# StefanDenn3r/Unsupervised_Anomaly_Detection_Brain_MRI

Hardware: AMD Instinct MI355X
Metric: MRI slices/sec VAE train step (128x128, bs=64) (higher is better)
Workload: dtype bf16x3; 1 GPU; BASELINE.json configs[1]: VAE 128x128x1 slices, batch 64 per GPU, fwd + bwd + TF-Adam (lr 1e-4, beta1 0.5), dropout 0.2, inter_res 8, zDim 128; global_batch=64, per_gpu_batch=64, parallelism=single

## Files before the change

unsupervised_anomaly_detection_brain_mri_amd/csrc/uad_conv16s.inc:

```

__device__ __forceinline__ float sum32_half(float v) {
    v += __uint_as_float(dpp_u32<0xB1>(__float_as_uint(v)));
    v += __uint_as_float(dpp_u32<0x4E>(__float_as_uint(v)));
    v += __uint_as_float(dpp_u32<0x141>(__float_as_uint(v)));
    v += __uint_as_float(dpp_u32<0x140>(__float_as_uint(v)));
    v += __uint_as_float((unsigned)__builtin_amdgcn_update_dpp(0, (int)__float_as_uint(v), 0x142, 0xa, 0xf, false));
    return v;
}
__device__ __forceinline__ bool sum32_valid(int lane) { return (lane & 16) != 0; }

__device__ __forceinline__ float xhalf_sum(float v) {
    const auto r = __builtin_amdgcn_permlane32_swap(__float_as_uint(v), __float_as_uint(v), false, false);
    return __uint_as_float(r[0]) + __uint_as_float(r[1]);
}
__device__ __forceinline__ unsigned xhalf_or(unsigned v) {
    const auto r = __builtin_amdgcn_permlane32_swap(v, v, false, false);
    return r[0] | r[1];
}

#ifndef UAD_D16S_NACC
#define UAD_D16S_NACC 1
#endif
template <int TH, int TW, int CST, int WGM, int WGN, int NPL = 2>
constexpr size_t conv5_d16s_lds_bytes(int epi) {
// ... 428 lines not shown
                    const int c = 8 * (r >> 2) + 4 * lh + (r & 3);
                    const float wfc = s_par[2 * BN + c];
                    fr[c] = t0;
                    fr[32 + c] = wfc * t1;
                    fr[64 + c] = wfc * t2;
                }
            }
        }
        float r0 = rec, r1 = dbf;
        r0 = sum32_half(r0); r1 = sum32_half(r1);
        if (lane == 16) { fr[96] = r1; fr[97] = r0; }
        __syncthreads();
        static_assert(TW == 16 && (TH == 8 || TH == 16), "partial-sum slots of the fused final epilogue are 8 x 16 tiles");
        const int slots_x = d.WS / 16;
        const size_t tile = ((size_t)n * (d.HS / 8) + ty0 / 8) * slots_x + tx0 / 16;
        if (tid < FL) {
            float t = 0.f;
#pragma unroll
            for (int w = 0; w < NW; ++w) t += s_red[w * FL + tid];
            if (tid == 97) a.ep.fin_rec_partial[tile] = t;
            else if (want_grad) a.ep.fin_red_partial[tile * 97 + tid] = t;
            if constexpr (TH == 16) {
                if (tid == 97) a.ep.fin_rec_partial[tile + slots_x] = 0.f;
                else if (want_grad) a.ep.fin_red_partial[(tile + slots_x) * 97 + tid] = 0.f;
            }
        }
        return;
    }
    if constexpr (BWD) {
        float* fr = s_red + wave * FL;
#pragma unroll
        for (int r = 0; r < 16; ++r) {
            const float t1 = sum32_half(s1[r]), t2 = sum32_half(s2[r]);
            if (l31 == 16) {
                const int c = 8 * (r >> 2) + 4 * lh + (r & 3);
                fr[c] = t1;
                fr[32 + c] = t2;
            }
        }
        __syncthreads();
// ... 63 lines not shown
```

unsupervised_anomaly_detection_brain_mri_amd/csrc/uad_gemm.hip:

```cpp
#include <type_traits>
#include "uad_kernels.h"
#include <hip/hip_ext.h>
#include <stdio.h>
#include <stdlib.h>
#include <string.h>
#include <map>
#include <array>
#include <string>
#include <vector>

#include "uad_gemm_common.h"

namespace {

constexpr int XF_LDS_CH = 512;

template <int BM, int BN, int BK, int WGM, int WGN, int KIND>
__global__ void __launch_bounds__(64 * WGM * WGN) conv_gemm_kernel(const ConvGemmArgs a) {
    constexpr int NT = 64 * WGM * WGN;
    constexpr int WTM = BM / WGM, WTN = BN / WGN;
    constexpr int FM = WTM / 32, FN = WTN / 32;
    static_assert(WTM % 32 == 0 && WTN % 32 == 0, "wave tile must be a multiple of the 32x32 MFMA");
    static_assert(BK % 8 == 0, "BK multiple of 8");
    constexpr int NKK = BK / 8;
// ... 2614 lines not shown
    for (int i = 0; i < n; ++i) v8 = v8 && pd.count[i] % 8 == 0 && pd.cb[i] % 8 == 0 && pd.cs[i] % 8 == 0;
    if (v8) hipLaunchKernelGGL(pack_weights_bf16_v8_kernel<3>, dim3((unsigned)((total / 8 + 255) / 256), 2), dim3(256), 0, st, params, w3_f, w3_d, pd);
    else hipLaunchKernelGGL(pack_weights_bf16_3p_kernel, dim3((unsigned)((total + 255) / 256)), dim3(256), 0, st, params, w3_f, w3_d, pd);
}

namespace {
void run_plan(const GemmPlan& p, ConvGemmArgs& a, bool f_type, float* ws, hipStream_t st) {
    const UadConvDesc& d = a.d;
    a.nsplit = 1; a.out_elems = p.out_elems;
    a.dbg = 0; a.dbgbuf = nullptr;
    if (p.path == PATH_SPATIAL) {
        float* out = a.Out;
        if (p.nsplit > 1) { a.Out = ws; a.nsplit = p.nsplit; a.out_final = out; }
        if (!(p.nsplit > 1 && p.inkernel && a.Wp16)) a.sk_counter = nullptr;
        dim3 grid((d.HS / p.sc.TH) * (d.WS / p.sc.TW), d.N, (a.Nn / p.sc.BN) * p.nsplit);
        if (a.Wp16) {
            if (f_type) {
                if (a.npl == 3) {
                    if (p.sc.BN == 64) {
                        if (a.xf.fb_bits || a.xf.fb_dxhat) { fprintf(stderr, "uad: final-backward on load runs on the 32-column instance (CA <= 32)\n"); abort(); }
                        if (a.xf.scale) launch_conv5_f16_v<8, 8, 16, 2, 2, 0, true, 3>(a, grid, st); else launch_conv5_f16_v<8, 8, 16, 2, 2, 0, false, 3>(a, grid, st);
                    } else launch_conv5_f16<8, 16, 16, 4, 1, 3>(a, grid, st);
                } else
                if (p.sc.BN == 64) launch_conv5_f16<8, 8, 32, 2, 2>(a, grid, st);
                else launch_conv5_f16<8, 16, 16, 4, 1>(a, grid, st);
            } else {
                const int cst = (a.CA % p.nsplit == 0) ? a.CA / p.nsplit : 0;
                constexpr bool seq = true;
                const bool lp = seq && conv5_d16s_takes(a);
                if (lp && ((p.sc.BN == 64 && (cst == 128 || cst == 64 || cst == 32)) || (p.sc.BN == 32 && (cst == 64 || cst == 32)))) launch_conv5_d16s_any(a, grid, p.sc.BN, cst, st);
                else if (a.npl == 3) { fprintf(stderr, "uad: a bf16x6 launch reached a kernel without the three-plane form (x6_route decides before run_plan)\n"); abort(); }
                else
                if (p.sc.BN == 64) {
                    if (seq && cst == 128) launch_conv5_d16<8, 8, 128, 2, 2>(a, grid, st);
                    else if (seq && cst == 64) launch_conv5_d16<8, 8, 64, 2, 2>(a, grid, st);
                    else if (seq && cst == 32) launch_conv5_d16<8, 8, 32, 2, 2>(a, grid, st);
                    else launch_conv5_bf16<8, 8, 32, 2, 2, KIND_D>(a, grid, st);
                } else if (seq && cst == 64) launch_conv5_d16<8, 16, 64, 4, 1>(a, grid, st);
                else if (seq && cst == 32) launch_conv5_d16<8, 16, 32, 4, 1>(a, grid, st);
                else if (p.sc.CK == 32) launch_conv5_bf16<8, 16, 32, 4, 1, KIND_D>(a, grid, st);
                else launch_conv5_bf16<8, 16, 16, 4, 1, KIND_D>(a, grid, st);
            }
        } else if (f_type) {
            if (p.sc.BN == 64) UAD_SPATIAL_LAUNCH((conv5_f_kernel<8, 8, 32, 2, 2>), grid, dim3(256), 0, st, a);
            else UAD_SPATIAL_LAUNCH((conv5_f_kernel<8, 16, 16, 4, 1>), grid, dim3(256), 0, st, a);
        } else {
            if (p.sc.BN == 64 && a.ep.kind != UAD_EPI_FINAL) UAD_SPATIAL_LAUNCH((conv5_d_kernel<8, 8, 32, 2, 2>), grid, dim3(256), 0, st, a);
            else if (p.sc.CK == 32 && a.ep.kind == UAD_EPI_FINAL && p.nsplit == 1 && a.Nn == 32) UAD_SPATIAL_LAUNCH((conv5_d_kernel<8, 16, 32, 4, 1, true>), grid, dim3(256), 0, st, a);
            else if (a.ep.kind == UAD_EPI_FINAL) { fprintf(stderr, "uad: fused final epilogue asked of an exact-fp32 launch that cannot run it (check uad_conv_d_can_fuse_final_f32 first)\n"); abort(); }
            else if (p.sc.CK == 32) UAD_SPATIAL_LAUNCH((conv5_d_kernel<8, 16, 32, 4, 1>), grid, dim3(256), 0, st, a);
            else UAD_SPATIAL_LAUNCH((conv5_d_kernel<8, 16, 16, 4, 1>), grid, dim3(256), 0, st, a);
        }
        if (p.nsplit > 1 && !a.sk_counter) {
            dim3 g2((p.out_rows + 63) / 64, (a.Nn + 63) / 64);
            hipLaunchKernelGGL(splitk_epilogue_kernel, g2, dim3(256), 0, st, ws, p.nsplit, p.out_elems, p.out_rows, a.Nn, a.ep, out);
        }
        return;
    }
    const int classes = f_type ? 1 : d.S * d.S;
    if (p.path == PATH_SPLITK) {
        float* out = a.Out;
        a.Out = ws; a.nsplit = p.nsplit;
        if (f_type) launch_gemm<KIND_F>(a, classes, st); else launch_gemm<KIND_D>(a, classes, st);
        dim3 grid((p.out_rows + 63) / 64, (a.Nn + 63) / 64);
        hipLaunchKernelGGL(splitk_epilogue_kernel, grid, dim3(256), 0, st, ws, p.nsplit, p.out_elems, p.out_rows, a.Nn, a.ep, out);
        return;
    }
// ... 244 lines not shown
```

unsupervised_anomaly_detection_brain_mri_amd/csrc/uad_kernels.h:

```cpp
#pragma once
#include <hip/hip_runtime.h>
#include <stdint.h>

struct UadConvDesc {
    int N;
    int HB, WB, CB;
    int HS, WS, CS;
    int KS, S, P;
};

struct UadXform {
    const float* scale = nullptr;
    const float* shift = nullptr;
    float alpha = 1.f;
    float mult = 1.f;
    const float* fb_dxhat = nullptr;
    const float* fb_wf = nullptr;
    const unsigned* fb_bits = nullptr;
};

enum { UAD_EPI_BIAS = 0, UAD_EPI_BWD_ACT = 1, UAD_EPI_FINAL = 2 };

struct UadGemmWs { float* ptr; size_t floats; unsigned* counters; int ncounters; };

// ... 7 lines not shown
    const float* eshift;
    float ealpha;
    float emult;
    float* colpart;
    const float* fin_wf;
    const float* fin_bf;
    const float* fin_x;
    float* fin_xhat;
    float* fin_l1;
    float* fin_rec_partial;
    float* fin_red_partial;
    float* fin_dc;
    unsigned* fin_bits;
    float* fin_dxhat;
    float fin_inv_batch;
};

void uad_launch_conv_f(const UadConvDesc& d, const float* big_in, UadXform xf, const float* W,
                       float* small_out, UadEpilogue ep, hipStream_t st, const float* Wpacked = nullptr,
                       UadGemmWs ws = UadGemmWs{nullptr, 0}, const unsigned short* Wp16 = nullptr, long long w16_plane = 0,
                       bool generic_bf16x3 = false, int planes16 = 2);
void uad_launch_conv_d(const UadConvDesc& d, const float* small_in, UadXform xf, const float* W,
                       float* big_out, UadEpilogue ep, hipStream_t st, const float* Wpacked = nullptr,
                       UadGemmWs ws = UadGemmWs{nullptr, 0}, const unsigned short* Wp16 = nullptr, long long w16_plane = 0,
                       bool generic_bf16x3 = false, int planes16 = 2);
void uad_launch_pack_weights_bf16(const float* params, unsigned short* w16_f, unsigned short* w16_d, const long long* offs,
                                  const int* cbs, const int* css, const int* taps, int n, hipStream_t st);
void uad_launch_pack_weights_bf16_3p(const float* params, unsigned short* w3_f, unsigned short* w3_d, const long long* offs,
                                     const int* cbs, const int* css, const int* taps, int n, hipStream_t st);
bool uad_conv_k3_takes(const UadConvDesc& d, bool f_type);
// ... 12 lines not shown
void uad_conv_plan_query(const UadConvDesc& d, bool f_type, bool have_pack, size_t ws_floats, int ncounters, int planes16, bool inst_ok, long long* out);
void uad_conv_w_plan_query(const UadConvDesc& d, bool math_bf16x3, int planes16, bool fbb, bool xa, bool xs, bool generic_bf16x3, bool defer_reduce, long long* out);
size_t uad_conv_w_partial_floats(const UadConvDesc& d);
bool uad_conv_w_supports_fb_bits(const UadConvDesc& d, bool math_bf16x3);
void uad_launch_conv_w(const UadConvDesc& d, const float* big, UadXform xfb, const float* small, UadXform xfs,
                       float* dW, float* partial, hipStream_t st, bool math_bf16x3 = false,
                       hipStream_t reduce_st = nullptr, hipEvent_t ev = nullptr, bool generic_bf16x3 = false, bool defer_reduce = false, int planes16 = 2);
void uad_launch_conv_w_reduce(const UadConvDesc& d, float* dW, float* partial, hipStream_t st, bool math_bf16x3);

void uad_launch_reduce_partials(const float* partial, int S, int L, float scale, float* out, hipStream_t st);
void uad_launch_bn_grad_finalize(const float* colpart, int T, int C, const float* gamma, float rstd,
                                 float* dgamma, float* dbeta, float* dbias, hipStream_t st, float* scratch = nullptr);
size_t uad_bn_grad_finalize_scratch_floats(int C);
void uad_launch_final_gradfin(const float* red, int C, const float* gamma, float rstd, float* dwf, float* dbf, float* dgamma, float* dbeta,
                              float* dbias, hipStream_t st);
void uad_launch_colsum(const float* g, int rows, int C, float* out, float* scratch, hipStream_t st);
size_t uad_colsum_scratch_floats(int rows, int C);

void uad_launch_conv_first_fwd(const UadConvDesc& d, const float* x, const float* W, const float* bias,
                               float* out, hipStream_t st);
size_t uad_conv_first_wgrad_partial_floats(const UadConvDesc& d);
void uad_launch_conv_first_wgrad(const UadConvDesc& d, const float* x, const float* g, float* dW,
                                 float* partial, hipStream_t st);

struct UadFinalArgs {
    int N, H, W, C;
    const float* c_last;
    const float* scale;
    const float* shift;
    float alpha;
// ... 123 lines not shown
void uad_launch_spatial_z_fwd(const float* c, const float* gamma, const float* beta, float rs0, float alpha, const float* mask, int rows,
                              int C, float* z, hipStream_t st);
int uad_spatial_z_bwd_blocks(int rows);
void uad_launch_spatial_z_bwd(const float* dz, const float* c, const float* gamma, const float* beta, float rs0, float alpha,
                              const float* mask, int rows, int C, float* dc, float* colpart, hipStream_t st);
struct UadRngJob { float* out; int per_sample; int kind; float rate; int stream; };
void uad_launch_rng_fill(const UadRngJob* jobs, int njobs, int n, unsigned long long seed, unsigned long long step, long long sample0,
                         hipStream_t st);
void uad_launch_clock_probe(unsigned long long* out, unsigned long long ticks, hipStream_t st);
void uad_launch_gather_slices(const float* src, const int* idx, int n, long long slice_elems, float* out, hipStream_t st);
void uad_launch_gather_mask(const unsigned char* labels, const int* idx, int n, long long slice_px, const unsigned char* lut,
                            float* out, hipStream_t st);
void uad_launch_mul(const float* x, const float* mask, float* y, size_t n, hipStream_t st);
void uad_launch_loss_finalize(const float* rec_partial, int n, int n_vae, int bps, const float* kl_per_sample,
                              float inv_batch, float rec_scale, float* rec_per_sample, float* scalars, hipStream_t st);

void uad_launch_optim(int kind, float* p, const float* g, float* s1, float* s2, size_t n, float lr, float momentum, float decay, float eps,
                      float gscale, hipStream_t st, const unsigned* fault = nullptr);
void uad_launch_adam(float* p, const float* g, float* m, float* v, size_t n, float lr_t, float beta1, float beta2,
                     float eps, float gscale, hipStream_t st, const unsigned* fault = nullptr);

void uad_launch_residual(const float* x, const float* xr, const float* mask, int n, int hw, int pos_only,
                         float prior_thresh, float* out, float* l1err, hipStream_t st);
```

unsupervised_anomaly_detection_brain_mri_amd/csrc/uad_misc.hip:

```cpp
#include "uad_kernels.h"
#include <stdint.h>

namespace {

__device__ __forceinline__ float wave_sum(float v) {
#pragma unroll
    for (int o = 32; o > 0; o >>= 1) v += __shfl_xor(v, o);
    return v;
}

typedef float v4f_nt __attribute__((ext_vector_type(4)));
template <int JL, int SL>
__global__ void __launch_bounds__(JL * SL) reduce_partials4_kernel(const float* __restrict__ partial, int S, int L, float scale, float* __restrict__ out) {
    __shared__ v4f_nt red[SL][JL];
    const int jl = threadIdx.x % JL, sl = threadIdx.x / JL;
    const int j4 = blockIdx.x * JL + jl, L4 = L >> 2;
    v4f_nt a0 = {0.f, 0.f, 0.f, 0.f}, a1 = a0, a2 = a0, a3 = a0;
    if (j4 < L4) {
        const v4f_nt* p = reinterpret_cast<const v4f_nt*>(partial) + j4;
        int s = sl;
        for (; s + 3 * SL < S; s += 4 * SL) {
            const v4f_nt v0 = __builtin_nontemporal_load(p + (size_t)s * L4), v1 = __builtin_nontemporal_load(p + (size_t)(s + SL) * L4);
            const v4f_nt v2 = __builtin_nontemporal_load(p + (size_t)(s + 2 * SL) * L4), v3 = __builtin_nontemporal_load(p + (size_t)(s + 3 * SL) * L4);
            a0 += v0; a1 += v1; a2 += v2; a3 += v3;
        }
        for (; s < S; s += SL) a0 += __builtin_nontemporal_load(p + (size_t)s * L4);
    }
    red[sl][jl] = (a0 + a1) + (a2 + a3);
    __syncthreads();
    if (sl == 0 && j4 < L4) {
        v4f_nt t = red[0][jl];
#pragma unroll
        for (int k = 1; k < SL; ++k) t += red[k][jl];
        reinterpret_cast<v4f_nt*>(out)[j4] = t * scale;
    }
}

template <int SL>
__global__ void __launch_bounds__(64 * SL) reduce_partials_kernel(const float* __restrict__ partial, int S, int L,
                                                                  float scale, float* __restrict__ out, int nt) {
    __shared__ float red[SL][64];
    const int jl = threadIdx.x & 63, sl = threadIdx.x >> 6;
    const int j = blockIdx.x * 64 + jl;
    float a0 = 0.f, a1 = 0.f, a2 = 0.f, a3 = 0.f;
    if (j < L) {
        int s = sl;
        if (nt) {
            for (; s + 3 * SL < S; s += 4 * SL) {
                a0 += __builtin_nontemporal_load(partial + (size_t)s * L + j);
                a1 += __builtin_nontemporal_load(partial + (size_t)(s + SL) * L + j);
                a2 += __builtin_nontemporal_load(partial + (size_t)(s + 2 * SL) * L + j);
                a3 += __builtin_nontemporal_load(partial + (size_t)(s + 3 * SL) * L + j);
            }
        }
        for (; s + 3 * SL < S; s += 4 * SL) {
            a0 += partial[(size_t)s * L + j];
            a1 += partial[(size_t)(s + SL) * L + j];
            a2 += partial[(size_t)(s + 2 * SL) * L + j];
            a3 += partial[(size_t)(s + 3 * SL) * L + j];
        }
        for (; s < S; s += SL) a0 += partial[(size_t)s * L + j];
    }
    red[sl][jl] = (a0 + a1) + (a2 + a3);
    __syncthreads();
    if (sl == 0 && j < L) {
        float t = 0.f;
#pragma unroll
        for (int k = 0; k < SL; ++k) t += red[k][jl];
        out[j] = t * scale;
    }
}

__global__ void __launch_bounds__(1024) bn_grad_finalize_kernel(const float* __restrict__ colpart, int T, int C,
                                                                const float* __restrict__ gamma, float rstd,
                                                                float* __restrict__ dgamma, float* __restrict__ dbeta,
                                                                float* __restrict__ dbias) {
    __shared__ float red[2][32][33];
    const int cl = threadIdx.x & 31, g = threadIdx.x >> 5;
// ... 61 lines not shown
        if (dbias) dbias[c] = gamma[c] * rstd * a1;
    }
}

__global__ void __launch_bounds__(256) final_gradfin_kernel(const float* __restrict__ red, int C, const float* __restrict__ gamma, float rstd,
                                                            float* __restrict__ dwf, float* __restrict__ dbf, float* __restrict__ dgamma,
                                                            float* __restrict__ dbeta, float* __restrict__ dbias) {
    for (int c = threadIdx.x; c < C; c += 256) {
        const float s1 = red[C + c], s2 = red[2 * C + c];
        dwf[c] = red[c];
        if (dbeta) dbeta[c] = s1;
        if (dgamma) dgamma[c] = s2 * rstd;
        if (dbias) dbias[c] = gamma[c] * rstd * s1;
    }
    if (threadIdx.x == 0) dbf[0] = red[3 * C];
}

__global__ void __launch_bounds__(256) colsum_kernel(const float* __restrict__ g, int rows, int C, int rows_per_chunk,
                                                     float* __restrict__ out) {
    __shared__ float red[8][33];
    const int cl = threadIdx.x & 31, rl = threadIdx.x >> 5;
    const int c = blockIdx.x * 32 + cl;
    const int r0 = blockIdx.y * rows_per_chunk;
    const int r1 = min(r0 + rows_per_chunk, rows);
    float s = 0.f;
    if (c < C)
        for (int r = r0 + rl; r < r1; r += 8) s += g[(size_t)r * C + c];
    red[rl][cl] = s;
    __syncthreads();
    if (rl == 0 && c < C) {
// ... 482 lines not shown
    __syncthreads();
    const int cq = threadIdx.x & 7, slot = threadIdx.x >> 3;
    first_dgrad_class<0, 0>(sg, W, cq, slot, sout);
    first_dgrad_class<0, 1>(sg, W, cq, slot, sout);
    first_dgrad_class<1, 0>(sg, W, cq, slot, sout);
    first_dgrad_class<1, 1>(sg, W, cq, slot, sout);
    __syncthreads();
    const int y = threadIdx.x >> 4, x = threadIdx.x & 15;
    first_dgrad_store(e, ((size_t)n * d.HB + ty0 + y) * d.WB + tx0 + x, sout[threadIdx.x]);
}

__global__ void __launch_bounds__(256) loss_finalize_kernel(const float* __restrict__ rec_partial, int n, int n_vae,
                                                            int bps, const float* __restrict__ kl, float inv_batch,
                                                            float rec_scale, float* __restrict__ rec_per_sample,
                                                            float* __restrict__ scalars) {
    __shared__ float sr[256], sc[256], sk[256];
    float ar = 0.f, ac = 0.f, ak = 0.f;
    for (int i = threadIdx.x; i < n; i += 256) {
        float r = 0.f;
        for (int b = 0; b < bps; ++b) r += rec_partial[(size_t)i * bps + b];
        rec_per_sample[i] = r;
        if (i < n_vae) { ar += r; if (kl) ak += kl[i]; }
        else ac += r;
    }
    sr[threadIdx.x] = ar;
    sc[threadIdx.x] = ac;
    sk[threadIdx.x] = ak;
    __syncthreads();
    if (threadIdx.x == 0) {
        float tr = 0.f, tc = 0.f, tk = 0.f;
        for (int i = 0; i < 256; ++i) { tr += sr[i]; tc += sc[i]; tk += sk[i]; }
        scalars[0] = rec_scale * (tr + tc) * inv_batch;
        scalars[1] = tk * inv_batch;
        scalars[2] = (tr + tk + tc) * inv_batch;
        scalars[3] = 0.f;
        scalars[4] = tr * inv_batch;
        scalars[5] = tc * inv_batch;
        scalars[6] = (tr + tk) * inv_batch;
        scalars[7] = 0.f;
    }
}

__global__ void __launch_bounds__(256) conv_first_dgrad_kernel(UadConvDesc d, const float* __restrict__ g,
                                                               const float* __restrict__ W,
                                                               const float* __restrict__ x,
                                                               const float* __restrict__ x_hat, float inv_batch,
                                                               float* __restrict__ anomaly, float* __restrict__ dx_out,
                                                               const float* __restrict__ dxhat, float* __restrict__ x_upd,
                                                               float restore_lr) {
    extern __shared__ __attribute__((aligned(16))) float sw[];
    const int CS = d.CS, KS = d.KS, S = d.S, P = d.P;
    for (int i = threadIdx.x; i < KS * KS * CS; i += 256) sw[i] = W[i];
    __syncthreads();
    const size_t pix = (size_t)blockIdx.x * 256 + threadIdx.x;
    const size_t total = (size_t)d.N * d.HB * d.WB;
// ... 259 lines not shown
        if ((L4 + 63) / 64 >= 256) hipLaunchKernelGGL((reduce_partials4_kernel<64, 8>), dim3((L4 + 63) / 64), dim3(512), 0, st, partial, S, L, scale, out);
        else if ((L4 + 31) / 32 >= 256) hipLaunchKernelGGL((reduce_partials4_kernel<32, 16>), dim3((L4 + 31) / 32), dim3(512), 0, st, partial, S, L, scale, out);
        else hipLaunchKernelGGL((reduce_partials4_kernel<16, 32>), dim3((L4 + 15) / 16), dim3(512), 0, st, partial, S, L, scale, out);
        return;
    }
    if (blocks >= 256 || S <= 8)
        hipLaunchKernelGGL((reduce_partials_kernel<4>), dim3(blocks), dim3(256), 0, st, partial, S, L, scale, out, nt);
    else
        hipLaunchKernelGGL((reduce_partials_kernel<16>), dim3(blocks), dim3(1024), 0, st, partial, S, L, scale, out, nt);
}

void uad_launch_final_gradfin(const float* red, int C, const float* gamma, float rstd, float* dwf, float* dbf, float* dgamma, float* dbeta,
                              float* dbias, hipStream_t st) {
    hipLaunchKernelGGL(final_gradfin_kernel, dim3(1), dim3(256), 0, st, red, C, gamma, rstd, dwf, dbf, dgamma, dbeta, dbias);
}
size_t uad_bn_grad_finalize_scratch_floats(int C) { return 64 + (size_t)((C + 31) / 32) * 32 * 64; }
void uad_launch_bn_grad_finalize(const float* colpart, int T, int C, const float* gamma, float rstd, float* dgamma,
                                 float* dbeta, float* dbias, hipStream_t st, float* scratch) {
    const int NB = T >= 2048 ? 32 : T >= 512 ? 16 : T >= 128 ? 8 : 1;
    if (scratch && NB > 1 && C <= 512) {
        hipLaunchKernelGGL(bn_grad_finalize2_kernel, dim3((C + 31) / 32, NB), dim3(1024), 0, st, colpart, T, C, gamma, rstd, dgamma, dbeta, dbias, scratch);
        return;
    }
    hipLaunchKernelGGL(bn_grad_finalize_kernel, dim3((C + 31) / 32), dim3(1024), 0, st, colpart, T, C, gamma, rstd,
                       dgamma, dbeta, dbias);
}

static inline int colsum_chunks(int rows, int C) {
    static const int cap_env = getenv("UAD_COLSUM_CHUNKS") ? atoi(getenv("UAD_COLSUM_CHUNKS")) : 0;
    int cap = cap_env > 0 ? cap_env : 1024;
// ... 162 lines not shown
```

unsupervised_anomaly_detection_brain_mri_amd/csrc/uad_model.hip:

```cpp
#include <math.h>
#include <stdarg.h>
#include <stdio.h>
#include <string.h>
#include <stdlib.h>

#include <string>
#include <vector>

#include <unistd.h>
#include "../../include/uad_hip.h"
#include "uad_allreduce.h"
#include "uad_kernels.h"

static thread_local std::string g_err;

int uad_fail(int code, const char* fmt, ...) {
    char buf[512];
    va_list ap;
    va_start(ap, fmt);
    vsnprintf(buf, sizeof buf, fmt, ap);
    va_end(ap);
    g_err = buf;
    return code;
}
// ... 60 lines not shown
    const float* dec_in0;
    bool restore;
    bool fb_on_load;
    float restore_tv, restore_lr;
    float restore_scale;
    float* restore_x;
    float* restore_grads;
    float *G0, *G1;
    float* dcb_keep;
    float* bott_xch; unsigned* bott_flags; unsigned bott_epoch;
    unsigned* bott_err_host; unsigned* bott_err_dev;
    unsigned* bott_fault;
    std::vector<unsigned> opt_epochs;
    bool fault_deferred;
    float* bnfin_scratch;
    float* bott_wpart;
    float *g_small[6];
    float *colpart, *wpartial, *colscratch, *red_partial, *rec_partial, *rec_ps, *scalars_own;
    size_t colpart_cap, wpartial_cap;
    int last_n, last_nuser;
    uad_io_t last_io;
    const float* x_eff;
    const float* mask_dec_eff;
    bool have_fwd;
    bool data_only;
    unsigned* fin_bits;
    float* fin_dxh;
    bool last_fin_bits;
    bool fwd_tail_is_loss;
    bool joined;
// ... 42 lines not shown
}
long long PLANE(const ConvLayer& L) { return (long long)L.d.KS * L.d.KS * L.d.CB * L.d.CS; }
float* Gr(uad_model* m, long long off) { return m->grads + off; }

UadXform bn_xform(uad_model* m, long long gamma, long long beta, float alpha) {
    UadXform x;
    x.scale = P(m, gamma); x.shift = P(m, beta); x.alpha = alpha; x.mult = 1.0f / sqrtf(1.0f + kBnEps);
    return x;
}
UadXform no_xform() { UadXform x; x.scale = nullptr; x.shift = nullptr; x.alpha = 1.f; x.mult = 1.f; return x; }
bool restore_fb_on_load(uad_model* m, int n) {
    if (!m->restore || !bf_mode(m)) return false;
    UadConvDesc d = m->dec.back().d; d.N = n;
    return uad_conv_f_supports_final_bwd(d, true, m->ws.floats);
}

UadEpilogue epi_bias(const float* bias, const float* mul = nullptr, const float* add = nullptr) {
    UadEpilogue e;
    memset(&e, 0, sizeof e);
    e.kind = UAD_EPI_BIAS; e.bias = bias; e.mul = mul; e.add = add;
    return e;
}
UadEpilogue epi_bwd(uad_model* m, const float* cprev, long long gamma, long long beta, float alpha) {
    UadEpilogue e;
    memset(&e, 0, sizeof e);
    e.kind = UAD_EPI_BWD_ACT; e.cprev = cprev; e.escale = P(m, gamma); e.eshift = P(m, beta); e.ealpha = alpha;
    e.emult = 1.0f / sqrtf(1.0f + kBnEps); e.colpart = m->colpart;
    return e;
}

// ... 233 lines not shown
    ALLOC(m->G0, maxact); ALLOC(m->G1, maxact);
    { float* fbw = nullptr; ALLOC(fbw, NB * H * Wd); m->fin_bits = reinterpret_cast<unsigned*>(fbw); ALLOC(m->fin_dxh, NB * H * Wd); }
    m->last_fin_bits = false;
    ALLOC(m->g_small[0], nflat); ALLOC(m->g_small[1], nz); ALLOC(m->g_small[2], nz); ALLOC(m->g_small[3], nz);
    ALLOC(m->g_small[4], nflat); ALLOC(m->g_small[5], nflat);
    ALLOC(m->dcb_keep, NB * ir * ir * m->cenc);
    ALLOC(m->bott_xch, NB * 4 * 2 * (size_t)cfg->zdim);
    { float* fl = nullptr; ALLOC(fl, NB * 4); m->bott_flags = reinterpret_cast<unsigned*>(fl); m->bott_epoch = 0; }
    m->bott_err_host = m->bott_err_dev = nullptr;
    { float* fw = nullptr; ALLOC(fw, 4); m->bott_fault = reinterpret_cast<unsigned*>(fw); m->opt_epochs.clear(); m->fault_deferred = false; }
    if (rc == UAD_OK && hipHostMalloc((void**)&m->bott_err_host, sizeof(unsigned), hipHostMallocMapped) == hipSuccess) {
        *m->bott_err_host = 0u;
        if (hipHostGetDevicePointer((void**)&m->bott_err_dev, m->bott_err_host, 0) != hipSuccess) m->bott_err_dev = nullptr;
    }
    ALLOC(m->bnfin_scratch, uad_bn_grad_finalize_scratch_floats(512));
    ALLOC(m->bott_wpart, NB * 4 * (2 * (size_t)m->cenc * m->cmid + m->cmid));
    size_t cp = 0;
    auto cp_need = [&](size_t rows, int classes, int C) { size_t v = ((rows + 63) / 64) * classes * 2 * C; if (v > cp) cp = v; };
    for (auto& L : m->enc) cp_need(NB * L.d.HS * L.d.WS, 4, L.d.CB);
    for (auto& L : m->dec) cp_need(NB * L.d.HS * L.d.WS, 1, L.d.CS);
    cp_need(NB * ir * ir, 1, m->cenc);
    if (NB * 4 * 2 * m->cenc > cp) cp = NB * 4 * 2 * m->cenc;
    if (gm) { size_t v = NB * ir * ir * 2 * m->cenc; if (v > cp) cp = v; }
    if (sp) { size_t v = (size_t)512 * 2 * m->cenc; if (v > cp) cp = v; }
    m->colpart_cap = cp; ALLOC(m->colpart, cp);
    for (int k = 0; k < 16; ++k) { m->cp_slot[k] = nullptr; ALLOC(m->cp_slot[k], cp); }
    m->ev_next = 0; m->side = nullptr;
    if (rc == UAD_OK && hipStreamCreateWithFlags(&m->side, hipStreamNonBlocking) != hipSuccess) rc = fail(UAD_ERR_HIP, "hipStreamCreate failed");
    size_t wp = 0;
    auto wp_need = [&](UadConvDesc d) { for (size_t nb = m->nmul; nb <= NB; nb += m->nmul) { d.N = (int)nb; size_t v = uad_conv_w_partial_floats(d); if (v > wp) wp = v; } };
// ... 297 lines not shown
        uad_launch_conv_f(dense_desc(n, m->flat, m->cfg.zdim), m->t, no_xform(), P(m, m->muw), m->mu_raw, epi_bias(P(m, m->mub)), st, nullptr, m->ws);
        uad_launch_conv_f(dense_desc(n, m->flat, m->cfg.zdim), m->t, no_xform(), P(m, m->sgw), m->ls_raw, epi_bias(P(m, m->sgb)), st, nullptr, m->ws);
        uad_launch_reparam_fwd(n, nu, m->cfg.zdim, m->mu_raw, m->ls_raw, io->mask_mu, io->mask_sigma,
                               cevae ? io->mask_mu_ce : nullptr, io->eps, m->mu, m->ls, m->sigma, m->z, m->kl, st);
        uad_launch_conv_f(dense_desc(n, m->cfg.zdim, m->flat), m->z, no_xform(), P(m, m->dw), m->dvec,
                          epi_bias(P(m, m->db), mask_dec), st, nullptr, m->ws);
    } else {
        uad_launch_conv_f(dense_desc(n, m->flat, m->cfg.zdim), m->t, no_xform(), P(m, m->muw), m->z,
                          epi_bias(P(m, m->mub), io->mask_mu), st, nullptr, m->ws);
        uad_launch_conv_f(dense_desc(n, m->cfg.zdim, m->flat), m->z, no_xform(), P(m, m->dw), m->dvec, epi_bias(P(m, m->db)), st, nullptr, m->ws);
    }
    uad_launch_conv_f(conv1x1_desc(n, ir, ir, m->cmid, m->cenc), m->dvec, no_xform(), P(m, m->rw), m->cb, epi_bias(P(m, m->rb)), st, nullptr, m->ws);
    }
    const ConvLayer& DL = m->dec.back();
    const int bps = uad_final_blocks_per_sample(m->cfg.height, m->cfg.width);
    bool fused_final = false, fin_bits_mode = false, restore_bits = false;
    for (size_t i = 0; i < m->dec.size(); ++i) {
        PROF(kDecF[i & 7]);
        UadConvDesc d = m->dec[i].d; d.N = n;
        const float* in = (i == 0) ? m->dec_in0 : m->dec[i - 1].c;
        UadXform xf = (i == 0) ? bn_xform(m, m->dbn_g, m->dbn_b, 0.0f)
                               : bn_xform(m, m->dec[i - 1].gamma, m->dec[i - 1].beta, kLrelu);
        UadEpilogue ep = epi_bias(P(m, m->dec[i].b));
        float* out = m->dec[i].c;
        const bool bfm = bf_mode(m);
        if (i + 1 == m->dec.size() && fuse_final_ok(m, d)) {
            fused_final = true;
            const bool restore_bwd = m->restore && want_backward;
            ep.kind = UAD_EPI_FINAL;
            ep.escale = P(m, DL.gamma); ep.eshift = P(m, DL.beta); ep.ealpha = kLrelu; ep.emult = 1.0f / sqrtf(1.0f + kBnEps);
            ep.fin_wf = P(m, m->fw); ep.fin_bf = P(m, m->fb); ep.fin_x = cevae ? xin : xtgt;
            ep.fin_xhat = (io->x_hat && !cevae) ? io->x_hat : m->xhat_own;
            ep.fin_l1 = cevae ? ((io->l1_map || io->l1_map_ce) ? m->l1_own : nullptr) : io->l1_map;
            ep.fin_rec_partial = m->rec_partial; ep.fin_red_partial = m->red_partial;
            ep.fin_dc = (want_backward && !restore_bwd) ? m->G0 : nullptr;
            ep.fin_bits = nullptr; ep.fin_dxhat = nullptr;
            if (ep.fin_dc && fin_bits_ok(m, d, want_backward)) {
                ep.fin_dc = nullptr; ep.fin_bits = m->fin_bits; ep.fin_dxhat = m->fin_dxh;
                fin_bits_mode = true;
            }
            ep.fin_inv_batch = 1.0f / (float)nu;
            static const bool no_rbits = getenv("UAD_NO_RESTORE_BITS") != nullptr;
            if (restore_bwd && bfm && !no_rbits && d.CB <= 32 && uad_conv_f_supports_final_bwd(d, true, m->ws.floats)) {
                ep.fin_bits = m->fin_bits; ep.fin_dxhat = m->fin_dxh;
                fin_bits_mode = true; restore_bits = true;
            }
            out = (restore_bwd && !restore_bits) ? DL.c : nullptr;
        }
        uad_launch_conv_d(d, in, xf, P(m, m->dec[i].w), out, ep, st, PKD(m, m->dec[i].w), m->ws, PK16D(m, m->dec[i].w), PLANE(m->dec[i]), false, planes_of(m));
    }
    UadFinalArgs fa;
    fa.N = n; fa.H = m->cfg.height; fa.W = m->cfg.width; fa.C = DL.d.CB;
    fa.c_last = DL.c; fa.scale = P(m, DL.gamma); fa.shift = P(m, DL.beta); fa.alpha = kLrelu;
    fa.mult = 1.0f / sqrtf(1.0f + kBnEps);
    fa.wf = P(m, m->fw); fa.bf = P(m, m->fb); fa.x = cevae ? xin : xtgt;
    fa.x_hat = (io->x_hat && !cevae) ? io->x_hat : m->xhat_own;
    fa.l1_map = cevae ? ((io->l1_map || io->l1_map_ce) ? m->l1_own : nullptr) : io->l1_map;
    fa.rec_partial = m->rec_partial;
    fa.d_c = want_backward ? m->G0 : nullptr;
    fa.red_partial = m->red_partial;
    fa.inv_batch = 1.0f / (float)nu;
// ... 4 lines not shown
        float* dc = fa.d_c; fa.d_c = nullptr;
        if (!fused_final) uad_launch_final_fwd_bwd(fa, st);
        uad_launch_tv_dxhat(xin, fa.x_hat, n, fa.H, fa.W, m->restore_scale, m->restore_tv, m->gm_dxhat, st);
        fa.d_c = dc; fa.dxhat_in = m->gm_dxhat;
        m->fb_on_load = fused_final && !restore_bits && restore_fb_on_load(m, n);
        if (!m->fb_on_load && !restore_bits) uad_launch_final_fwd_bwd(fa, st);
    } else {
        PROF(want_backward ? "final.fwd+bwd" : "final.fwd"); uad_launch_final_fwd_bwd(fa, st);
    }
    if (m->restore) {
    } else if (gm) {
        PROF("loss.finalize");
        uad_launch_gm_loss_finalize(m->rec_partial, n, bps, m->gm_loc_loss, ir * ir, 1.0f / (float)nu,
                                    io->rec_per_sample ? io->rec_per_sample : m->rec_ps,
                                    io->scalars ? io->scalars : m->scalars_own, st);
    } else {
    PROF("loss.finalize");
    uad_launch_loss_finalize(m->rec_partial, n, nu, bps, vae ? m->kl : nullptr, 1.0f / (float)nu, cevae ? 0.5f : 1.0f,
                             io->rec_per_sample ? io->rec_per_sample : m->rec_ps,
                             io->scalars ? io->scalars : m->scalars_own, st);
    }
    if (cevae) {
        const size_t xe = (size_t)nu * m->cfg.height * m->cfg.width * m->cfg.channels, xb = xe * sizeof(float);
        if (io->x_hat) HIP_TRY(hipMemcpyAsync(io->x_hat, m->xhat_own, xb, hipMemcpyDeviceToDevice, st));
        if (io->x_hat_ce) HIP_TRY(hipMemcpyAsync(io->x_hat_ce, m->xhat_own + xe, xb, hipMemcpyDeviceToDevice, st));
        if (io->l1_map) HIP_TRY(hipMemcpyAsync(io->l1_map, m->l1_own, xb, hipMemcpyDeviceToDevice, st));
        if (io->l1_map_ce) HIP_TRY(hipMemcpyAsync(io->l1_map_ce, m->l1_own + xe, xb, hipMemcpyDeviceToDevice, st));
    }
    const size_t zb = (gm || sp) ? 0 : (size_t)nu * m->cfg.zdim * sizeof(float);
    if (sp && io->z_mu) hipMemcpyAsync(io->z_mu, m->gm_h, (size_t)nu * ir * ir * m->cenc * sizeof(float), hipMemcpyDeviceToDevice, st);
    if (!gm && !sp && io->z_mu) hipMemcpyAsync(io->z_mu, vae ? m->mu : m->z, zb, hipMemcpyDeviceToDevice, st);
    if (vae && io->z_log_sigma) hipMemcpyAsync(io->z_log_sigma, m->ls, zb, hipMemcpyDeviceToDevice, st);
    if (vae && io->z_sigma) hipMemcpyAsync(io->z_sigma, m->sigma, zb, hipMemcpyDeviceToDevice, st);
    m->last_n = n; m->last_nuser = nu; m->last_io = *io; m->have_fwd = want_backward != 0;
    m->x_eff = xin; m->mask_dec_eff = mask_dec; m->data_only = want_backward == 2;
    m->last_fused_final = fused_final && !(m->restore && want_backward);
    m->last_fin_bits = fin_bits_mode;
    m->fwd_tail_is_loss = !m->restore && !gm && !cevae && !io->z_mu && !io->z_log_sigma && !io->z_sigma;
    HIP_TRY(hipGetLastError());
    return UAD_OK;
}

static int sk_counters(const uad_model* m) { return (bf_mode(m) && m->ws.counters) ? m->ws.ncounters : 0; }
static hipEvent_t next_event(uad_model* m) {
    if (m->ev_next == m->sync_events.size()) {
        hipEvent_t e;
        if (hipEventCreateWithFlags(&e, hipEventDisableTiming | hipEventDisableSystemFence) != hipSuccess)
            (void)hipEventCreateWithFlags(&e, hipEventDisableTiming);
        m->sync_events.push_back(e);
    }
    return m->sync_events[m->ev_next++];
}
static void edge(uad_model* m, hipStream_t from, hipStream_t to) {
// ... 34 lines not shown
        { static const bool anyo = getenv("UAD_NO_ANYORDER") == nullptr;
          if (anyo && pg && bf && last && m->fwd_tail_is_loss && !m->prof_on) uad_conv_w_any_order_next(true);
          m->fwd_tail_is_loss = false; }
        if (pg) { PROF(kDecW[i & 7]); uad_launch_conv_w(d, g, fbb ? gbits : no_xform(), in, bn_xform(m, ig, ib, ia), Gr(m, m->dec[i].w), m->wp_slot[i], st, bf, nullptr, nullptr, false, true, planes_of(m)); }
        uad_conv_w_any_order_next(false);
        { static const bool anyo = getenv("UAD_NO_ANYORDER") == nullptr; if (anyo && pg) uad_conv_any_order_next(true); }
        { PROF(kDecD[i & 7]); UadEpilogue e = epi_bwd(m, in, ig, ib, ia); e.colpart = cp;
          const bool fb = m->restore && m->fb_on_load && last;
          UadXform gx = fbb ? gbits : no_xform();
          if (fb) { gx = bn_xform(m, DL.gamma, DL.beta, kLrelu); gx.fb_dxhat = m->gm_dxhat; gx.fb_wf = P(m, m->fw); }
          uad_launch_conv_f(d, fb ? DL.c : g, gx, P(m, m->dec[i].w), gn, e, st, PKF(m, m->dec[i].w), m->ws, PK16F(m, m->dec[i].w), PLANE(m->dec[i]), false, planes_of(m));
          uad_conv_any_order_next(false); }
        if (pg) edge(m, st, sd);
        if (pg && last) {
            PROF_ON("final.gradfin", sd);
            uad_launch_reduce_partials(m->red_partial, T, L, 1.0f, m->colscratch, sd);
            uad_launch_final_gradfin(m->colscratch, C, P(m, DL.gamma), rstd, Gr(m, m->fw), Gr(m, m->fb), Gr(m, DL.gamma), Gr(m, DL.beta), Gr(m, DL.b), sd);
        }
        if (pg) { PROF_ON("bn.gradfin", sd); uad_launch_conv_w_reduce(d, Gr(m, m->dec[i].w), m->wp_slot[i], sd, bf); uad_launch_bn_grad_finalize(cp, uad_conv_f_tiles(d, true, m->ws.floats, sk_counters(m), planes_of(m)), d.CS, P(m, ig), rstd, Gr(m, ig), Gr(m, ib), ibias >= 0 ? Gr(m, ibias) : nullptr, sd, m->bnfin_scratch); }
        float* tsw = g; g = gn; gn = tsw;
    }
    m->G0 = g; m->G1 = gn;
    if (join_now) join_side(m, st);
    return UAD_OK;
}

static int backward_bottleneck(uad_model* m, hipStream_t st, bool join_now) {
    const int n = m->last_n, nu = m->last_nuser;
    const bool vae = m->cfg.arch != UAD_ARCH_AE;
    const bool cevae = m->cfg.arch == UAD_ARCH_CEVAE;
    const bool pg = !m->data_only;
    const int ir = m->cfg.inter_res, zd = m->cfg.zdim;
// ... 633 lines not shown
```

Baseline: 78530 slices/s.

## Fold loss finalize and final grad reduction into last-arriver workgroups

Adds ticket counters so that the last workgroup to finish the fused final-layer conv computes the per-sample reconstruction sums and loss scalars in place, removing a separate loss_finalize launch. On the backward side stream, the reduce_partials and final_gradfin kernels are merged into one kernel where the last block finalizes the gradients. This trims two small kernel launches per step. In exchange it adds atomic ticket traffic and a serialized tail inside the conv kernel. It also drops the any-order hint that depended on the forward tail being a loss kernel.

```diff
diff --git a/unsupervised_anomaly_detection_brain_mri_amd/csrc/uad_conv16s.inc b/unsupervised_anomaly_detection_brain_mri_amd/csrc/uad_conv16s.inc
--- a/unsupervised_anomaly_detection_brain_mri_amd/csrc/uad_conv16s.inc
+++ b/unsupervised_anomaly_detection_brain_mri_amd/csrc/uad_conv16s.inc
@@ -466,16 +466,28 @@
         static_assert(TW == 16 && (TH == 8 || TH == 16), "partial-sum slots of the fused final epilogue are 8 x 16 tiles");
         const int slots_x = d.WS / 16;
         const size_t tile = ((size_t)n * (d.HS / 8) + ty0 / 8) * slots_x + tx0 / 16;
+        unsigned* const ticket = a.ep.fin_ticket;
         if (tid < FL) {
             float t = 0.f;
 #pragma unroll
             for (int w = 0; w < NW; ++w) t += s_red[w * FL + tid];
-            if (tid == 97) a.ep.fin_rec_partial[tile] = t;
-            else if (want_grad) a.ep.fin_red_partial[tile * 97 + tid] = t;
+            if (tid == 97) {
+                if (ticket) __hip_atomic_store(a.ep.fin_rec_partial + tile, t, __ATOMIC_RELAXED, __HIP_MEMORY_SCOPE_AGENT);
+                else a.ep.fin_rec_partial[tile] = t;
+            } else if (want_grad) a.ep.fin_red_partial[tile * 97 + tid] = t;
             if constexpr (TH == 16) {
-                if (tid == 97) a.ep.fin_rec_partial[tile + slots_x] = 0.f;
-                else if (want_grad) a.ep.fin_red_partial[(tile + slots_x) * 97 + tid] = 0.f;
-            }
+                if (tid == 97) {
+                    if (ticket) __hip_atomic_store(a.ep.fin_rec_partial + tile + slots_x, 0.f, __ATOMIC_RELAXED, __HIP_MEMORY_SCOPE_AGENT);
+                    else a.ep.fin_rec_partial[tile + slots_x] = 0.f;
+                } else if (want_grad) a.ep.fin_red_partial[(tile + slots_x) * 97 + tid] = 0.f;
+            }
+        }
+        if (ticket) {
+            static_assert(NT == 256, "uad_loss_totals is written for loss_finalize_kernel's 256 threads");
+            const int nwg = (int)(gridDim.x * gridDim.y * gridDim.z);
+            if (sk_last_arriver(ticket, nwg, reinterpret_cast<int*>(s_red), tid))
+                uad_loss_totals<true>(a.ep.fin_rec_partial, a.ep.fin_n, a.ep.fin_nvae, a.ep.fin_bps, a.ep.fin_kl, a.ep.fin_inv_batch, a.ep.fin_rec_scale,
+                                      a.ep.fin_rec_ps, a.ep.fin_scalars, s_fx, tid);
         }
         return;
     }
diff --git a/unsupervised_anomaly_detection_brain_mri_amd/csrc/uad_gemm.hip b/unsupervised_anomaly_detection_brain_mri_amd/csrc/uad_gemm.hip
--- a/unsupervised_anomaly_detection_brain_mri_amd/csrc/uad_gemm.hip
+++ b/unsupervised_anomaly_detection_brain_mri_amd/csrc/uad_gemm.hip
@@ -2652,6 +2652,7 @@
         if (p.nsplit > 1) { a.Out = ws; a.nsplit = p.nsplit; a.out_final = out; }
         if (!(p.nsplit > 1 && p.inkernel && a.Wp16)) a.sk_counter = nullptr;
         dim3 grid((d.HS / p.sc.TH) * (d.WS / p.sc.TW), d.N, (a.Nn / p.sc.BN) * p.nsplit);
+        bool fin_totals_done = false;
         if (a.Wp16) {
             if (f_type) {
                 if (a.npl == 3) {
@@ -2666,7 +2667,7 @@
                 const int cst = (a.CA % p.nsplit == 0) ? a.CA / p.nsplit : 0;
                 constexpr bool seq = true;
                 const bool lp = seq && conv5_d16s_takes(a);
-                if (lp && ((p.sc.BN == 64 && (cst == 128 || cst == 64 || cst == 32)) || (p.sc.BN == 32 && (cst == 64 || cst == 32)))) launch_conv5_d16s_any(a, grid, p.sc.BN, cst, st);
+                if (lp && ((p.sc.BN == 64 && (cst == 128 || cst == 64 || cst == 32)) || (p.sc.BN == 32 && (cst == 64 || cst == 32)))) { launch_conv5_d16s_any(a, grid, p.sc.BN, cst, st); fin_totals_done = true; }
                 else if (a.npl == 3) { fprintf(stderr, "uad: a bf16x6 launch reached a kernel without the three-plane form (x6_route decides before run_plan)\n"); abort(); }
                 else
                 if (p.sc.BN == 64) {
@@ -2689,6 +2690,9 @@
             else if (p.sc.CK == 32) UAD_SPATIAL_LAUNCH((conv5_d_kernel<8, 16, 32, 4, 1>), grid, dim3(256), 0, st, a);
             else UAD_SPATIAL_LAUNCH((conv5_d_kernel<8, 16, 16, 4, 1>), grid, dim3(256), 0, st, a);
         }
+        if (a.ep.kind == UAD_EPI_FINAL && a.ep.fin_ticket && !fin_totals_done)
+            uad_launch_loss_finalize(a.ep.fin_rec_partial, a.ep.fin_n, a.ep.fin_nvae, a.ep.fin_bps, a.ep.fin_kl, a.ep.fin_inv_batch, a.ep.fin_rec_scale,
+                                     a.ep.fin_rec_ps, a.ep.fin_scalars, st);
         if (p.nsplit > 1 && !a.sk_counter) {
             dim3 g2((p.out_rows + 63) / 64, (a.Nn + 63) / 64);
             hipLaunchKernelGGL(splitk_epilogue_kernel, g2, dim3(256), 0, st, ws, p.nsplit, p.out_elems, p.out_rows, a.Nn, a.ep, out);
diff --git a/unsupervised_anomaly_detection_brain_mri_amd/csrc/uad_kernels.h b/unsupervised_anomaly_detection_brain_mri_amd/csrc/uad_kernels.h
--- a/unsupervised_anomaly_detection_brain_mri_amd/csrc/uad_kernels.h
+++ b/unsupervised_anomaly_detection_brain_mri_amd/csrc/uad_kernels.h
@@ -45,6 +45,12 @@
     unsigned* fin_bits;
     float* fin_dxhat;
     float fin_inv_batch;
+    unsigned* fin_ticket;
+    int fin_n, fin_nvae, fin_bps;
+    const float* fin_kl;
+    float fin_rec_scale;
+    float* fin_rec_ps;
+    float* fin_scalars;
 };
 
 void uad_launch_conv_f(const UadConvDesc& d, const float* big_in, UadXform xf, const float* W,
@@ -87,6 +93,8 @@
 size_t uad_bn_grad_finalize_scratch_floats(int C);
 void uad_launch_final_gradfin(const float* red, int C, const float* gamma, float rstd, float* dwf, float* dbf, float* dgamma, float* dbeta,
                               float* dbias, hipStream_t st);
+void uad_launch_reduce_final_gradfin(const float* partial, int S, int C, const float* gamma, float rstd, float* red, float* dwf, float* dbf,
+                                     float* dgamma, float* dbeta, float* dbias, unsigned* ticket, hipStream_t st);
 void uad_launch_colsum(const float* g, int rows, int C, float* out, float* scratch, hipStream_t st);
 size_t uad_colsum_scratch_floats(int rows, int C);
 
@@ -240,6 +248,41 @@
 void uad_launch_mul(const float* x, const float* mask, float* y, size_t n, hipStream_t st);
 void uad_launch_loss_finalize(const float* rec_partial, int n, int n_vae, int bps, const float* kl_per_sample,
                               float inv_batch, float rec_scale, float* rec_per_sample, float* scalars, hipStream_t st);
+#ifdef __HIPCC__
+template <bool COHERENT>
+__device__ __forceinline__ void uad_loss_totals(const float* rec_partial, int n, int n_vae, int bps, const float* kl, float inv_batch, float rec_scale,
+                                                float* rec_per_sample, float* scalars, float* s3, int tid) {
+    float* sr = s3; float* sc = s3 + 256; float* sk = s3 + 512;
+    float ar = 0.f, ac = 0.f, ak = 0.f;
+    for (int i = tid; i < n; i += 256) {
+        float r = 0.f;
+        for (int b = 0; b < bps; ++b) {
+            const float* p = rec_partial + (size_t)i * bps + b;
+            if constexpr (COHERENT) r += __hip_atomic_load(p, __ATOMIC_RELAXED, __HIP_MEMORY_SCOPE_AGENT);
+            else r += *p;
+        }
+        rec_per_sample[i] = r;
+        if (i < n_vae) { ar += r; if (kl) ak += kl[i]; }
+        else ac += r;
+    }
+    sr[tid] = ar;
+    sc[tid] = ac;
+    sk[tid] = ak;
+    __syncthreads();
+    if (tid == 0) {
+        float tr = 0.f, tc = 0.f, tk = 0.f;
+        for (int i = 0; i < 256; ++i) { tr += sr[i]; tc += sc[i]; tk += sk[i]; }
+        scalars[0] = rec_scale * (tr + tc) * inv_batch;
+        scalars[1] = tk * inv_batch;
+        scalars[2] = (tr + tk + tc) * inv_batch;
+        scalars[3] = 0.f;
+        scalars[4] = tr * inv_batch;
+        scalars[5] = tc * inv_batch;
+        scalars[6] = (tr + tk) * inv_batch;
+        scalars[7] = 0.f;
+    }
+}
+#endif
 
 void uad_launch_optim(int kind, float* p, const float* g, float* s1, float* s2, size_t n, float lr, float momentum, float decay, float eps,
                       float gscale, hipStream_t st, const unsigned* fault = nullptr);
diff --git a/unsupervised_anomaly_detection_brain_mri_amd/csrc/uad_misc.hip b/unsupervised_anomaly_detection_brain_mri_amd/csrc/uad_misc.hip
--- a/unsupervised_anomaly_detection_brain_mri_amd/csrc/uad_misc.hip
+++ b/unsupervised_anomaly_detection_brain_mri_amd/csrc/uad_misc.hip
@@ -37,11 +37,7 @@
 }
 
 template <int SL>
-__global__ void __launch_bounds__(64 * SL) reduce_partials_kernel(const float* __restrict__ partial, int S, int L,
-                                                                  float scale, float* __restrict__ out, int nt) {
-    __shared__ float red[SL][64];
-    const int jl = threadIdx.x & 63, sl = threadIdx.x >> 6;
-    const int j = blockIdx.x * 64 + jl;
+__device__ __forceinline__ float reduce_partials_lane(const float* __restrict__ partial, int S, int L, int j, int sl, int nt) {
     float a0 = 0.f, a1 = 0.f, a2 = 0.f, a3 = 0.f;
     if (j < L) {
         int s = sl;
@@ -61,7 +57,15 @@
         }
         for (; s < S; s += SL) a0 += partial[(size_t)s * L + j];
     }
-    red[sl][jl] = (a0 + a1) + (a2 + a3);
+    return (a0 + a1) + (a2 + a3);
+}
+template <int SL>
+__global__ void __launch_bounds__(64 * SL) reduce_partials_kernel(const float* __restrict__ partial, int S, int L,
+                                                                  float scale, float* __restrict__ out, int nt) {
+    __shared__ float red[SL][64];
+    const int jl = threadIdx.x & 63, sl = threadIdx.x >> 6;
+    const int j = blockIdx.x * 64 + jl;
+    red[sl][jl] = reduce_partials_lane<SL>(partial, S, L, j, sl, nt);
     __syncthreads();
     if (sl == 0 && j < L) {
         float t = 0.f;
@@ -153,6 +157,41 @@
         if (dbias) dbias[c] = gamma[c] * rstd * s1;
     }
     if (threadIdx.x == 0) dbf[0] = red[3 * C];
+}
+template <int SL>
+__global__ void __launch_bounds__(64 * SL) reduce_final_gradfin_kernel(const float* __restrict__ partial, int S, int C, const float* __restrict__ gamma,
+                                                                       float rstd, float* red, float* __restrict__ dwf, float* __restrict__ dbf,
+                                                                       float* __restrict__ dgamma, float* __restrict__ dbeta, float* __restrict__ dbias,
+                                                                       unsigned* ticket) {
+    __shared__ float lred[SL][64];
+    __shared__ int s_last;
+    const int L = 3 * C + 1;
+    const int jl = threadIdx.x & 63, sl = threadIdx.x >> 6;
+    const int j = blockIdx.x * 64 + jl;
+    lred[sl][jl] = reduce_partials_lane<SL>(partial, S, L, j, sl, 1);
+    __syncthreads();
+    if (sl == 0 && j < L) {
+        float t = 0.f;
+#pragma unroll
+        for (int k = 0; k < SL; ++k) t += lred[k][jl];
+        __hip_atomic_store(red + j, t, __ATOMIC_RELAXED, __HIP_MEMORY_SCOPE_AGENT);
+    }
+    __builtin_amdgcn_s_waitcnt(0);
+    __builtin_amdgcn_fence(__ATOMIC_RELEASE, "workgroup");
+    __syncthreads();
+    if (threadIdx.x == 0) s_last = (__hip_atomic_fetch_add(ticket, 1u, __ATOMIC_RELAXED, __HIP_MEMORY_SCOPE_AGENT) == gridDim.x - 1u);
+    __syncthreads();
+    if (!s_last) return;
+    if (threadIdx.x == 0) __hip_atomic_store(ticket, 0u, __ATOMIC_RELAXED, __HIP_MEMORY_SCOPE_AGENT);
+    for (int c = threadIdx.x; c < C; c += 64 * SL) {
+        const float s1 = __hip_atomic_load(red + C + c, __ATOMIC_RELAXED, __HIP_MEMORY_SCOPE_AGENT);
+        const float s2 = __hip_atomic_load(red + 2 * C + c, __ATOMIC_RELAXED, __HIP_MEMORY_SCOPE_AGENT);
+        dwf[c] = __hip_atomic_load(red + c, __ATOMIC_RELAXED, __HIP_MEMORY_SCOPE_AGENT);
+        if (dbeta) dbeta[c] = s1;
+        if (dgamma) dgamma[c] = s2 * rstd;
+        if (dbias) dbias[c] = gamma[c] * rstd * s1;
+    }
+    if (threadIdx.x == 0) dbf[0] = __hip_atomic_load(red + 3 * C, __ATOMIC_RELAXED, __HIP_MEMORY_SCOPE_AGENT);
 }
 
 __global__ void __launch_bounds__(256) colsum_kernel(const float* __restrict__ g, int rows, int C, int rows_per_chunk,
@@ -665,31 +704,8 @@
                                                             int bps, const float* __restrict__ kl, float inv_batch,
                                                             float rec_scale, float* __restrict__ rec_per_sample,
                                                             float* __restrict__ scalars) {
-    __shared__ float sr[256], sc[256], sk[256];
-    float ar = 0.f, ac = 0.f, ak = 0.f;
-    for (int i = threadIdx.x; i < n; i += 256) {
-        float r = 0.f;
-        for (int b = 0; b < bps; ++b) r += rec_partial[(size_t)i * bps + b];
-        rec_per_sample[i] = r;
-        if (i < n_vae) { ar += r; if (kl) ak += kl[i]; }
-        else ac += r;
-    }
-    sr[threadIdx.x] = ar;
-    sc[threadIdx.x] = ac;
-    sk[threadIdx.x] = ak;
-    __syncthreads();
-    if (threadIdx.x == 0) {
-        float tr = 0.f, tc = 0.f, tk = 0.f;
-        for (int i = 0; i < 256; ++i) { tr += sr[i]; tc += sc[i]; tk += sk[i]; }
-        scalars[0] = rec_scale * (tr + tc) * inv_batch;
-        scalars[1] = tk * inv_batch;
-        scalars[2] = (tr + tk + tc) * inv_batch;
-        scalars[3] = 0.f;
-        scalars[4] = tr * inv_batch;
-        scalars[5] = tc * inv_batch;
-        scalars[6] = (tr + tk) * inv_batch;
-        scalars[7] = 0.f;
-    }
+    __shared__ float s3[768];
+    uad_loss_totals<false>(rec_partial, n, n_vae, bps, kl, inv_batch, rec_scale, rec_per_sample, scalars, s3, (int)threadIdx.x);
 }
 
 __global__ void __launch_bounds__(256) conv_first_dgrad_kernel(UadConvDesc d, const float* __restrict__ g,
@@ -979,6 +995,17 @@
                               float* dbias, hipStream_t st) {
     hipLaunchKernelGGL(final_gradfin_kernel, dim3(1), dim3(256), 0, st, red, C, gamma, rstd, dwf, dbf, dgamma, dbeta, dbias);
 }
+void uad_launch_reduce_final_gradfin(const float* partial, int S, int C, const float* gamma, float rstd, float* red, float* dwf, float* dbf,
+                                     float* dgamma, float* dbeta, float* dbias, unsigned* ticket, hipStream_t st) {
+    const int L = 3 * C + 1, blocks = (L + 63) / 64;
+    if (blocks >= 256 || (L % 4 == 0 && L >= 1024)) {
+        uad_launch_reduce_partials(partial, S, L, 1.0f, red, st);
+        uad_launch_final_gradfin(red, C, gamma, rstd, dwf, dbf, dgamma, dbeta, dbias, st);
+    } else if (S <= 8)
+        hipLaunchKernelGGL((reduce_final_gradfin_kernel<4>), dim3(blocks), dim3(256), 0, st, partial, S, C, gamma, rstd, red, dwf, dbf, dgamma, dbeta, dbias, ticket);
+    else
+        hipLaunchKernelGGL((reduce_final_gradfin_kernel<16>), dim3(blocks), dim3(1024), 0, st, partial, S, C, gamma, rstd, red, dwf, dbf, dgamma, dbeta, dbias, ticket);
+}
 size_t uad_bn_grad_finalize_scratch_floats(int C) { return 64 + (size_t)((C + 31) / 32) * 32 * 64; }
 void uad_launch_bn_grad_finalize(const float* colpart, int T, int C, const float* gamma, float rstd, float* dgamma,
                                  float* dbeta, float* dbias, hipStream_t st, float* scratch) {
diff --git a/unsupervised_anomaly_detection_brain_mri_amd/csrc/uad_model.hip b/unsupervised_anomaly_detection_brain_mri_amd/csrc/uad_model.hip
--- a/unsupervised_anomaly_detection_brain_mri_amd/csrc/uad_model.hip
+++ b/unsupervised_anomaly_detection_brain_mri_amd/csrc/uad_model.hip
@@ -98,6 +98,7 @@
     std::vector<unsigned> opt_epochs;
     bool fault_deferred;
     float* bnfin_scratch;
+    unsigned* la_tickets;
     float* bott_wpart;
     float *g_small[6];
     float *colpart, *wpartial, *colscratch, *red_partial, *rec_partial, *rec_ps, *scalars_own;
@@ -170,6 +171,8 @@
     UadConvDesc d = m->dec.back().d; d.N = n;
     return uad_conv_f_supports_final_bwd(d, true, m->ws.floats);
 }
+
+bool last_arriver_on() { static const bool on = getenv("UAD_NO_LAST_ARRIVER") == nullptr; return on; }
 
 UadEpilogue epi_bias(const float* bias, const float* mul = nullptr, const float* add = nullptr) {
     UadEpilogue e;
@@ -433,6 +436,7 @@
         if (hipHostGetDevicePointer((void**)&m->bott_err_dev, m->bott_err_host, 0) != hipSuccess) m->bott_err_dev = nullptr;
     }
     ALLOC(m->bnfin_scratch, uad_bn_grad_finalize_scratch_floats(512));
+    { float* tk = nullptr; ALLOC(tk, 4); m->la_tickets = reinterpret_cast<unsigned*>(tk); }
     ALLOC(m->bott_wpart, NB * 4 * (2 * (size_t)m->cenc * m->cmid + m->cmid));
     size_t cp = 0;
     auto cp_need = [&](size_t rows, int classes, int C) { size_t v = ((rows + 63) / 64) * classes * 2 * C; if (v > cp) cp = v; };
@@ -760,7 +764,7 @@
     }
     const ConvLayer& DL = m->dec.back();
     const int bps = uad_final_blocks_per_sample(m->cfg.height, m->cfg.width);
-    bool fused_final = false, fin_bits_mode = false, restore_bits = false;
+    bool fused_final = false, fin_bits_mode = false, restore_bits = false, loss_in_launch = false;
     for (size_t i = 0; i < m->dec.size(); ++i) {
         PROF(kDecF[i & 7]);
         UadConvDesc d = m->dec[i].d; d.N = n;
@@ -791,6 +795,13 @@
                 ep.fin_bits = m->fin_bits; ep.fin_dxhat = m->fin_dxh;
                 fin_bits_mode = true; restore_bits = true;
             }
+            if (fin_bits_mode && !m->restore && !gm && last_arriver_on()) {
+                ep.fin_ticket = m->la_tickets; ep.fin_n = n; ep.fin_nvae = nu; ep.fin_bps = bps;
+                ep.fin_kl = vae ? m->kl : nullptr; ep.fin_rec_scale = cevae ? 0.5f : 1.0f;
+                ep.fin_rec_ps = io->rec_per_sample ? io->rec_per_sample : m->rec_ps;
+                ep.fin_scalars = io->scalars ? io->scalars : m->scalars_own;
+                loss_in_launch = true;
+            }
             out = (restore_bwd && !restore_bits) ? DL.c : nullptr;
         }
         uad_launch_conv_d(d, in, xf, P(m, m->dec[i].w), out, ep, st, PKD(m, m->dec[i].w), m->ws, PK16D(m, m->dec[i].w), PLANE(m->dec[i]), false, planes_of(m));
@@ -825,6 +836,7 @@
         uad_launch_gm_loss_finalize(m->rec_partial, n, bps, m->gm_loc_loss, ir * ir, 1.0f / (float)nu,
                                     io->rec_per_sample ? io->rec_per_sample : m->rec_ps,
                                     io->scalars ? io->scalars : m->scalars_own, st);
+    } else if (loss_in_launch) {
     } else {
     PROF("loss.finalize");
     uad_launch_loss_finalize(m->rec_partial, n, nu, bps, vae ? m->kl : nullptr, 1.0f / (float)nu, cevae ? 0.5f : 1.0f,
@@ -847,7 +859,7 @@
     m->x_eff = xin; m->mask_dec_eff = mask_dec; m->data_only = want_backward == 2;
     m->last_fused_final = fused_final && !(m->restore && want_backward);
     m->last_fin_bits = fin_bits_mode;
-    m->fwd_tail_is_loss = !m->restore && !gm && !cevae && !io->z_mu && !io->z_log_sigma && !io->z_sigma;
+    m->fwd_tail_is_loss = !m->restore && !gm && !cevae && !io->z_mu && !io->z_log_sigma && !io->z_sigma && !loss_in_launch;
     HIP_TRY(hipGetLastError());
     return UAD_OK;
 }
@@ -912,8 +924,12 @@
         if (pg) edge(m, st, sd);
         if (pg && last) {
             PROF_ON("final.gradfin", sd);
-            uad_launch_reduce_partials(m->red_partial, T, L, 1.0f, m->colscratch, sd);
-            uad_launch_final_gradfin(m->colscratch, C, P(m, DL.gamma), rstd, Gr(m, m->fw), Gr(m, m->fb), Gr(m, DL.gamma), Gr(m, DL.beta), Gr(m, DL.b), sd);
+            if (last_arriver_on()) {
+                uad_launch_reduce_final_gradfin(m->red_partial, T, C, P(m, DL.gamma), rstd, m->colscratch, Gr(m, m->fw), Gr(m, m->fb), Gr(m, DL.gamma), Gr(m, DL.beta), Gr(m, DL.b), m->la_tickets + 1, sd);
+            } else {
+                uad_launch_reduce_partials(m->red_partial, T, L, 1.0f, m->colscratch, sd);
+                uad_launch_final_gradfin(m->colscratch, C, P(m, DL.gamma), rstd, Gr(m, m->fw), Gr(m, m->fb), Gr(m, DL.gamma), Gr(m, DL.beta), Gr(m, DL.b), sd);
+            }
         }
         if (pg) { PROF_ON("bn.gradfin", sd); uad_launch_conv_w_reduce(d, Gr(m, m->dec[i].w), m->wp_slot[i], sd, bf); uad_launch_bn_grad_finalize(cp, uad_conv_f_tiles(d, true, m->ws.floats, sk_counters(m), planes_of(m)), d.CS, P(m, ig), rstd, Gr(m, ig), Gr(m, ib), ibias >= 0 ? Gr(m, ibias) : nullptr, sd, m->bnfin_scratch); }
         float* tsw = g; g = gn; gn = tsw;
```

After: 78240 slices/s. No clear change (-0.4%).
